# epruesse/SINA

Measured on AMD Instinct MI355X. Metric: aligned sequences/sec (whole node), 100k full-length 16S vs SILVA-NR-scale ref, higher is better.
Workload: dtype f32

## Files before the change

### sina_amd/csrc/graph_build.hip

```cpp
#include <algorithm>
#include <cstring>
#include <type_traits>

#include "common.h"
#include "ctx.h"

namespace sina_hip {
namespace {

#ifndef SINA_GRAPH_THREADS
#define SINA_GRAPH_THREADS 512
#endif
#ifndef SINA_GRAPH_MINWAVES
#define SINA_GRAPH_MINWAVES 8
#endif
constexpr int kGT = SINA_GRAPH_THREADS;
constexpr uint32_t kNoPrev = 0xFFFFu;
constexpr int kMaxFam = kFamilyMax;
constexpr int kSz = kBuiltWords;
#ifndef SINA_GRAPH_KTC
#define SINA_GRAPH_KTC 128
#endif
#ifndef SINA_GRAPH_TNW
#define SINA_GRAPH_TNW 512
#endif
constexpr int kTC = SINA_GRAPH_KTC;
constexpr int kTNW = SINA_GRAPH_TNW;
static_assert(kTC % 64 == 0 && kTC < 255 && kTNW >= 32 && kTNW % 2 == 0, "tile geometry");
static_assert((kMaxFam * (kTC / 64) + SINA_GRAPH_THREADS / 64 - 1) / (SINA_GRAPH_THREADS / 64) <= 64, "far-entry flags of a wave fit 64 bits");

#ifdef SINA_DP_PROFILE
__device__ unsigned long long g_graph_prof[16];
#define GP_DECL unsigned long long gp_[16] = {}; unsigned long long gt_ = __builtin_amdgcn_s_memtime();
#define GP(i) { const unsigned long long t_ = __builtin_amdgcn_s_memtime(); gp_[i] += t_ - gt_; gt_ = t_; }
#define GP_FLUSH if (threadIdx.x == 0) { for (int i_ = 0; i_ < 16; i_++) atomicAdd(&g_graph_prof[i_], gp_[i_]); }
#else
#define GP_DECL
#define GP(i)
#define GP_FLUSH
#endif

struct GraphArgs {
    const uint32_t *ref_ab;
    const uint64_t *ref_off;
    const uint32_t *fam_ids;
    const uint64_t *fam_off;
    const uint64_t *pred_off;
    const float *wtab;
    uint4 *rec;
    uint32_t *node_pos;
    uint32_t *succ_min;
    uint32_t *far_mark;
    uint32_t *pred;
    uint32_t *sizes;
    uint32_t width, ncap;
    uint32_t tile_bytes;
    uint32_t bitmap_off;
    uint32_t member_off;
    uint32_t member_cap;
    uint32_t fam_cap;
    int W;
    int want_smin;
    uint2 *reach;
    float kappa64;
};

struct Member {
    uint64_t beg;
    uint32_t len;
    uint32_t cur, curn;
    uint32_t carry, carryn;
    uint32_t id;
};
static_assert(sizeof(Member) == 32, "LDS layout");
constexpr uint32_t kOCpos = 0;
constexpr uint32_t kONbase = kOCpos + 4 * kTC;
constexpr uint32_t kOPres = kONbase + 4 * (kTC + 2);
constexpr uint32_t kOWA = kOPres + 4 * kTC;
constexpr uint32_t kOWC = kOWA + 4 * kTNW;
constexpr uint32_t kOWD = kOWC + 4 * kTNW;
constexpr uint32_t kOWB = (kOWD + 4 * kTNW + 7) & ~7u;
constexpr uint32_t kOLi = kOWB + 8 * kTNW;
constexpr uint32_t kONn = kOLi + 32 * kTC;
constexpr uint32_t kONfar = kONn + kTC;
constexpr uint32_t kOMask = kONfar + kTNW;
constexpr uint32_t kONcol = kOMask + kTNW;
constexpr uint32_t kOE = (kONcol + kTNW + 15) & ~15u;

template <typename In, typename Out>
__device__ uint32_t block_exscan(const In *in, Out *out, uint32_t n, uint32_t *tmp) {
    const uint32_t tid = threadIdx.x;
    const uint32_t chunk = (n + kGT - 1) / kGT;
    const uint32_t b = min(n, tid * chunk), e = min(n, b + chunk);
    uint32_t s = 0;
    for (uint32_t i = b; i < e; i++) s += (uint32_t)in[i];
    uint32_t x = s;
    const int lane = tid & 63, wave = tid >> 6;
#pragma unroll
    for (int off = 1; off < 64; off <<= 1) {
        const uint32_t y = __shfl_up(x, off);
        if (lane >= off) x += y;
    }
    if (lane == 63) tmp[wave] = x;
    __syncthreads();
    uint32_t base = 0, total = 0;
    for (int w = 0; w < kGT / 64; w++) {
        if (w < wave) base += tmp[w];
        total += tmp[w];
    }
    uint32_t run = base + x - s;
    __syncthreads();
    for (uint32_t i = b; i < e; i++) {
        const uint32_t v = (uint32_t)in[i];
        out[i] = (Out)run;
        run += v;
    }
    __syncthreads();
    return total;
}

template <typename Get, typename Out>
__device__ uint32_t block_exscan_f(uint32_t n, Get get, Out *out, uint32_t *tmp) {
    const uint32_t tid = threadIdx.x;
    const uint32_t chunk = (n + kGT - 1) / kGT;
    const uint32_t b = min(n, tid * chunk), e = min(n, b + chunk);
    uint32_t s = 0;
    for (uint32_t i = b; i < e; i++) s += get(i);
    uint32_t x = s;
    const int lane = tid & 63, wave = tid >> 6;
#pragma unroll
    for (int off = 1; off < 64; off <<= 1) {
        const uint32_t y = __shfl_up(x, off);
        if (lane >= off) x += y;
    }
    if (lane == 63) tmp[wave] = x;
    __syncthreads();
    uint32_t base = 0, total = 0;
    for (int w = 0; w < kGT / 64; w++) {
        if (w < wave) base += tmp[w];
        total += tmp[w];
    }
    uint32_t run = base + x - s;
    __syncthreads();
    for (uint32_t i = b; i < e; i++) {
        const uint32_t v = get(i);
        out[i] = (Out)run;
        run += v;
    }
    __syncthreads();
    return total;
}

__device__ __attribute__((noinline)) void fill_tile(const uint32_t *__restrict__ ref_ab, uint32_t bitmap_off, uint32_t member_off,
                                                    uint32_t nwords, uint32_t n_tasks, uint32_t c0, uint32_t tc) {
    extern __shared__ __attribute__((aligned(16))) unsigned char smem[];
    uint32_t *cposT = reinterpret_cast<uint32_t *>(smem + kOCpos);
    uint32_t *presT = reinterpret_cast<uint32_t *>(smem + kOPres);
    uint16_t *eE = reinterpret_cast<uint16_t *>(smem + kOE);
    const uint32_t *bitmap = reinterpret_cast<const uint32_t *>(smem + bitmap_off);
    const uint16_t *wrank = reinterpret_cast<const uint16_t *>(bitmap + nwords);
    Member *mb = reinterpret_cast<Member *>(smem + member_off);
    constexpr uint32_t kEAbsent = 0x00FFu, kEFirst = 1u << 13;
    constexpr uint32_t kCH = kTC / 64, kNW = kGT / 64;
    const uint32_t wave = (uint32_t)__builtin_amdgcn_readfirstlane((int)(threadIdx.x >> 6));
    const uint32_t lane = threadIdx.x & 63u;
    auto rank = [&](uint32_t pos) -> uint32_t {
        return (uint32_t)wrank[pos >> 5] + __popc(bitmap[pos >> 5] & ((1u << (pos & 31)) - 1u));
    };
        for (uint32_t t4 = wave; t4 < n_tasks; t4 += 8 * kNW) {
            uint32_t abv[8];
#pragma unroll
            for (int u = 0; u < 8; u++) {
                const uint32_t task = t4 + (uint32_t)u * kNW;
                abv[u] = 0xFFFFFFFFu;
                if (task < n_tasks) {
                    const uint32_t j = task / kCH;
                    const uint32_t cur = (uint32_t)__builtin_amdgcn_readfirstlane((int)mb[j].cur);
                    const uint32_t len = (uint32_t)__builtin_amdgcn_readfirstlane((int)mb[j].len);
                    const uint64_t beg = mb[j].beg;
                    const uint64_t begs = ((uint64_t)(uint32_t)__builtin_amdgcn_readfirstlane((int)(uint32_t)(beg >> 32)) << 32) |
                                          (uint32_t)__builtin_amdgcn_readfirstlane((int)(uint32_t)beg);
                    const uint32_t i = cur + (task % kCH) * 64u + lane;
                    if (i < len) abv[u] = ref_ab[begs + i];
                }
            }
#pragma unroll
            for (int u = 0; u < 8; u++) {
                const uint32_t task = t4 + (uint32_t)u * kNW;
                if (task >= n_tasks) continue;
                const uint32_t j = task / kCH, slot0 = (task % kCH) * 64u, slot = slot0 + lane;
                const uint32_t cur = (uint32_t)__builtin_amdgcn_readfirstlane((int)mb[j].cur);
                uint32_t ev = kEAbsent;
                if (abv[u] != 0xFFFFFFFFu) {
                    const uint32_t ab = abv[u];
                    const uint32_t pos = ab & 0xFFFFFFu;
                    const uint32_t c = rank(pos) - c0;
                    if (c < tc) {
                        const uint32_t m = (ab >> 24) & 0x1Fu;
                        ev = c | (m << 8) | (cur + slot == 0 ? kEFirst : 0u);
                        atomicOr(&presT[c], 1u << m);
                        cposT[c] = pos;
                    }
                }
                eE[j * (uint32_t)kTC + slot] = (uint16_t)ev;
                const uint32_t n_in = (uint32_t)__popcll(__builtin_amdgcn_ballot_w64(ev != kEAbsent));
                if (n_in && lane == 0) atomicMax(&mb[j].curn, cur + slot0 + n_in);
            }
        }
}

__device__ __forceinline__ uint32_t node_of_entry(uint32_t ev) {
    extern __shared__ __attribute__((aligned(16))) unsigned char smem[];
    const uint32_t *nbaseT = reinterpret_cast<const uint32_t *>(smem + kONbase);
    const uint32_t *presT = reinterpret_cast<const uint32_t *>(smem + kOPres);
    const uint8_t *liOf = smem + kOLi;
    const uint32_t c = ev & 0xFFu, m = (ev >> 8) & 31u;
    const uint32_t b = nbaseT[c];
    return b + liOf[b + __popc(presT[c] & ((1u << m) - 1u))];
}
__global__ void __launch_bounds__(kGT) __attribute__((amdgpu_waves_per_eu(SINA_GRAPH_MINWAVES, SINA_GRAPH_MINWAVES))) family_graph_kernel(GraphArgs a) {
    extern __shared__ __attribute__((aligned(16))) unsigned char smem[];
    __shared__ uint32_t s_tmp[kGT / 64 + 8];
    const uint32_t q = blockIdx.x, tid = threadIdx.x;
    const uint32_t nwords = (a.width + 31) / 32;
    const uint64_t f0 = a.fam_off[q];
    const uint32_t F = (uint32_t)(a.fam_off[q + 1] - f0);
    uint32_t *cposT = reinterpret_cast<uint32_t *>(smem + kOCpos);
    uint32_t *nbaseT = reinterpret_cast<uint32_t *>(smem + kONbase);
    uint32_t *presT = reinterpret_cast<uint32_t *>(smem + kOPres);
    uint32_t *wA = reinterpret_cast<uint32_t *>(smem + kOWA);
    uint32_t *wC = reinterpret_cast<uint32_t *>(smem + kOWC);
    uint32_t *wD = reinterpret_cast<uint32_t *>(smem + kOWD);
    unsigned long long *wB = reinterpret_cast<unsigned long long *>(smem + kOWB);
    uint8_t *liOf = smem + kOLi;
    uint8_t *nn = smem + kONn;
    uint8_t *nfarN = smem + kONfar;
    uint8_t *maskN = smem + kOMask;
    uint8_t *ncolN = smem + kONcol;
    uint16_t *eE = reinterpret_cast<uint16_t *>(smem + kOE);
    uint32_t *bitmap = reinterpret_cast<uint32_t *>(smem + a.bitmap_off);
    uint16_t *wrank = reinterpret_cast<uint16_t *>(bitmap + nwords);
    Member *mb = reinterpret_cast<Member *>(smem + a.member_off);
    constexpr uint32_t kEFirst = 1u << 13;
    constexpr uint32_t kCH = kTC / 64, kNW = kGT / 64;
    const uint32_t wave = (uint32_t)__builtin_amdgcn_readfirstlane((int)(threadIdx.x >> 6));
    const uint32_t lane = threadIdx.x & 63u;
    const uint32_t n_tasks = F * kCH;

    uint32_t *sz = a.sizes + kSz * (size_t)q;
    for (uint32_t j = tid; j < F; j += kGT) {
        const uint32_t id = a.fam_ids[f0 + j];
        mb[j].id = id;
        mb[j].beg = a.ref_off[id];
        mb[j].len = (uint32_t)(a.ref_off[id + 1] - a.ref_off[id]);
        mb[j].cur = mb[j].curn = 0;
        mb[j].carry = mb[j].carryn = kNoPrev;
    }
    for (uint32_t i = tid; i < nwords; i += kGT) bitmap[i] = 0;
    __syncthreads();
    GP_DECL

    for (uint32_t j0 = 0; j0 < F; j0 += 8) {
        uint32_t maxlen = 0;
#pragma unroll
        for (int u = 0; u < 8; u++) maxlen = max(maxlen, j0 + u < F ? mb[j0 + u].len : 0u);
        for (uint32_t i = tid; i < maxlen; i += kGT) {
            uint32_t ab[8];
#pragma unroll
            for (int u = 0; u < 8; u++)
                ab[u] = (j0 + u < F && i < mb[j0 + u].len) ? a.ref_ab[mb[j0 + u].beg + i] : 0xFFFFFFFFu;
#pragma unroll
            for (int u = 0; u < 8; u++)
                if (ab[u] != 0xFFFFFFFFu) {
                    const uint32_t pos = ab[u] & 0xFFFFFFu;
                    atomicOr(&bitmap[pos >> 5], 1u << (pos & 31));
                }
        }
    }
    __syncthreads();
    GP(0)
    {
        const uint32_t chunk = (nwords + kGT - 1) / kGT;
        const uint32_t b = min(nwords, tid * chunk), e = min(nwords, b + chunk);
        uint32_t s = 0;
        for (uint32_t i = b; i < e; i++) s += __popc(bitmap[i]);
        uint32_t x = s;
        const int lane = tid & 63, wave = tid >> 6;
#pragma unroll
        for (int off = 1; off < 64; off <<= 1) {
            const uint32_t y = __shfl_up(x, off);
            if (lane >= off) x += y;
        }
        if (lane == 63) s_tmp[wave] = x;
        __syncthreads();
        uint32_t base = 0, total = 0;
        for (int w = 0; w < kGT / 64; w++) {
            if (w < wave) base += s_tmp[w];
            total += s_tmp[w];
        }
        uint32_t run = base + x - s;
        for (uint32_t i = b; i < e; i++) {
            wrank[i] = (uint16_t)run;
            run += __popc(bitmap[i]);
        }
        if (tid == 0) s_tmp[kGT / 64] = total;
    }
    __syncthreads();
    const uint32_t NC = s_tmp[kGT / 64];
    if (NC > 65535u) {
        if (tid == 0) {
            sz[0] = NC;
            sz[1] = sz[2] = 0;
            sz[3] = 2;
        }
        return;
    }
    auto rank = [&](uint32_t pos) -> uint32_t {
        return (uint32_t)wrank[pos >> 5] + __popc(bitmap[pos >> 5] & ((1u << (pos & 31)) - 1u));
    };
    uint4 *rec = a.rec + (size_t)q * a.ncap;
    uint32_t *node_pos = a.node_pos + (size_t)q * a.ncap;
    uint32_t *smin = a.succ_min + (size_t)q * a.ncap;
    uint32_t *last = a.far_mark + (size_t)q * a.ncap;
    uint32_t *pred = a.pred + a.pred_off[q];
    const float *wt = a.wtab + (size_t)F * (kMaxFam + 1);
    uint32_t N = 0, E = 0;
    GP(1)

    for (uint32_t c0 = 0; c0 < NC; c0 += kTC) {
        const uint32_t tc = min((uint32_t)kTC, NC - c0);
        for (uint32_t i = tid; i < (uint32_t)kTC; i += kGT) presT[i] = 0;
        __syncthreads();
        GP(2)
        fill_tile(a.ref_ab, a.bitmap_off, a.member_off, nwords, n_tasks, c0, tc);
        __syncthreads();
        for (uint32_t c = tid; c < tc; c += kGT) nn[c] = (uint8_t)__popc(presT[c]);
        __syncthreads();
        GP(3)
        const uint32_t tn = block_exscan(nn, nbaseT, tc, s_tmp);
        if (tid == 0) nbaseT[tc] = tn;
        for (uint32_t ln = tid; ln < tn; ln += kGT)
            if (N + ln < a.ncap) {
                last[N + ln] = 0;
                if (a.want_smin) smin[N + ln] = 0xFFFFFFFFu;
            }
        __syncthreads();
        GP(5)
        uint32_t te = 0;
        for (uint32_t ca = 0; ca < tc;) {
            const uint32_t w0 = nbaseT[ca];
            uint32_t cb = tc;
            if (tn - w0 > (uint32_t)kTNW) {
                uint32_t lo = ca + 1, hi = tc;
                while (lo < hi) {
                    const uint32_t mid = (lo + hi + 1) / 2;
                    if (nbaseT[mid] - w0 <= (uint32_t)kTNW) lo = mid;
                    else hi = mid - 1;
                }
                cb = lo;
            }
            const uint32_t wn = nbaseT[cb] - w0;
            for (uint32_t i = tid; i < wn; i += kGT) {
                wA[i] = 0;
                wB[i] = 0;
                wC[i] = 0xFFFFFFFFu;
                nfarN[i] = 0;
            }
            __syncthreads();
            for (uint32_t task = wave; task < n_tasks; task += kNW) {
                const uint32_t j = task / kCH, slot = (task % kCH) * 64u + lane;
                const uint32_t ev = eE[j * (uint32_t)kTC + slot];
                const uint32_t c = ev & 0xFFu;
                if (c >= ca && c < cb) {
                    const uint32_t m = (ev >> 8) & 31u;
                    atomicMin(&wC[nbaseT[c] + __popc(presT[c] & ((1u << m) - 1u)) - w0], j);
                }
            }
            __syncthreads();
            for (uint32_t c = ca + tid; c < cb; c += kGT) {
                const uint32_t base = nbaseT[c], k = nn[c];
                uint32_t pp = presT[c];
                for (uint32_t x = 0; x < k; x++) {
                    const uint32_t mj = wC[base - w0 + x];
                    uint32_t r = 0;
                    for (uint32_t y = 0; y < k; y++) r += (wC[base - w0 + y] < mj) ? 1u : 0u;
                    liOf[base + x] = (uint8_t)r;
                    maskN[base - w0 + r] = (uint8_t)(__ffs(pp) - 1);
                    ncolN[base - w0 + r] = (uint8_t)c;
                    pp &= pp - 1u;
                }
            }
            __syncthreads();
            GP(4)
            auto node_of = [&](uint32_t ev) -> uint32_t { return node_of_entry(ev); };
            unsigned long long farbits = 0;
            {
                uint32_t it = 0;
                for (uint32_t task = wave; task < n_tasks; task += kNW, it++) {
                    const uint32_t j = task / kCH, slot = (task % kCH) * 64u + lane;
                    const uint32_t ev = eE[j * (uint32_t)kTC + slot];
                    const uint32_t c = ev & 0xFFu;
                    const bool mine = c >= ca && c < cb;
                    const uint32_t ln = mine ? node_of(ev) : 0u;
                    uint32_t lnp = __shfl_up(ln, 1);
                    const bool left_mine = __shfl_up(mine ? 1 : 0, 1) != 0;
                    if (!mine) continue;
                    const uint32_t node = N + ln;
                    const bool first = (ev & kEFirst) != 0;
                    atomicAdd(&wA[ln - w0], first ? 1u : 0x10001u);
                    if (mb[j].cur + slot + 1 == mb[j].curn) mb[j].carryn = node;
                    if (!first) {
                        if (slot && (lane == 0 || !left_mine)) lnp = node_of(eE[j * (uint32_t)kTC + slot - 1]);
                        const uint32_t pn = slot ? N + lnp : mb[j].carry;
                        const uint32_t d = node - pn;
                        if (d <= 64u) atomicOr(&wB[ln - w0], 1ull << (d - 1u));
                        else farbits |= 1ull << it;
                    }
                }
            }
            for (uint32_t i = tid; i < wn; i += kGT) wC[i] = 0xFFFFFFFFu;
            __syncthreads();
            GP(6)
            const uint32_t te_w = block_exscan_f(wn, [&](uint32_t i) { return wA[i] >> 16; }, wD, s_tmp);
            while (__syncthreads_or(farbits != 0 ? 1 : 0)) {
                uint32_t it = 0;
                for (uint32_t task = wave; task < n_tasks; task += kNW, it++) {
                    if (!((farbits >> it) & 1ull)) continue;
                    const uint32_t j = task / kCH, slot = (task % kCH) * 64u + lane;
                    const uint32_t ln = node_of(eE[j * (uint32_t)kTC + slot]);
                    const uint32_t pn = slot ? N + node_of(eE[j * (uint32_t)kTC + slot - 1]) : mb[j].carry;
                    atomicMin(&wC[ln - w0], pn);
                }
                __syncthreads();
                it = 0;
                for (uint32_t task = wave; task < n_tasks; task += kNW, it++) {
                    if (!((farbits >> it) & 1ull)) continue;
                    const uint32_t j = task / kCH, slot = (task % kCH) * 64u + lane;
                    const uint32_t ln = node_of(eE[j * (uint32_t)kTC + slot]);
                    const uint32_t pn = slot ? N + node_of(eE[j * (uint32_t)kTC + slot - 1]) : mb[j].carry;
                    if (wC[ln - w0] == pn) farbits &= ~(1ull << it);
                }
                __syncthreads();
                for (uint32_t i = tid; i < wn; i += kGT) {
                    const uint32_t v = wC[i];
                    if (v == 0xFFFFFFFFu) continue;
                    const uint32_t node = N + w0 + i;
                    if (node < a.ncap) {
                        pred[E + te + wD[i] + nfarN[i]] = v;
                        if (a.want_smin) atomicMin(&smin[v], cposT[ncolN[i]]);
                        atomicMax(&last[v], node);
                    }
                    nfarN[i]++;
                    wC[i] = 0xFFFFFFFFu;
                }
            }
            for (uint32_t i = tid; i < wn; i += kGT) {
                const uint32_t node = N + w0 + i;
                if (node >= a.ncap) continue;
                const uint32_t seg = E + te + wD[i];
                const uint32_t pos = cposT[ncolN[i]];
                uint32_t np = nfarN[i];
                unsigned long long bits = wB[i];
                while (bits) {
                    const uint32_t hi = 63u - (uint32_t)__clzll((long long)bits);
                    bits ^= 1ull << hi;
                    const uint32_t pa = node - (hi + 1u);
                    pred[seg + np] = pa;
                    np++;
                    if (a.want_smin) atomicMin(&smin[pa], pos);
                    atomicMax(&last[pa], node);
                }
                uint4 r;
                r.x = seg;
                r.y = __float_as_uint(wt[wA[i] & 0xFFFFu]);
                r.z = (np & 0xFFu) | ((uint32_t)maskN[i] << 8);
                r.w = kRowNone;
                rec[node] = r;
                node_pos[node] = pos;
            }
            te += te_w;
            ca = cb;
            __syncthreads();
        }
        for (uint32_t j = tid; j < F; j += kGT) {
            mb[j].cur = mb[j].curn;
            mb[j].carry = mb[j].carryn;
        }
        N += tn;
        E += te;
        __syncthreads();
        GP(7)
    }
    if (N > a.ncap || N > 65535u) {
        if (tid == 0) {
            sz[0] = N;
            sz[1] = sz[2] = 0;
            sz[3] = 2;
        }
        return;
    }
    GP(8)
    const uint32_t seg_len = dp_slot_segment(N);
    const uint32_t n_seg = (N + seg_len - 1) / seg_len;
    uint32_t *codeL = reinterpret_cast<uint32_t *>(smem);
    const bool in_lds = (size_t)N * 4 <= a.tile_bytes;
    if (tid == 0) s_tmp[kGT / 64 + 1] = 0xFFFFFFFFu;
    __syncthreads();
    for (uint32_t i = tid; i < N; i += kGT) {
        uint32_t z = rec[i].z;
        const uint32_t l = last[i];
        if (l == 0) {
            z |= kRecSink;
            atomicMin(&s_tmp[kGT / 64 + 1], i);
            if (a.want_smin) smin[i] = 1000000u;
        }
        if (l > i && l - i > (uint32_t)kFarLds) z |= kRecFence;
        rec[i].z = z;
        if (in_lds) codeL[i] = l | ((z & kRecSink) ? (1u << 30) : 0u) | ((z & kRecFence) ? (1u << 31) : 0u);
    }
    __syncthreads();
    GP(9)
    if (tid < n_seg) {
        auto walk = [&](auto kslots) {
            constexpr int K = decltype(kslots)::value;
            uint32_t fa[K];
#pragma unroll
            for (int x = 0; x < K; x++) fa[x] = (x < a.W) ? 0u : 0xFFFFFFFFu;
            uint32_t nsp = 0;
            const uint32_t b = tid * seg_len, e = min(N, b + seg_len);
            for (uint32_t m = b; m < e; m++) {
                uint32_t l, sink, fence;
                if (in_lds) {
                    const uint32_t cd = codeL[m];
                    l = cd & 0xFFFFu;
                    sink = cd & (1u << 30);
                    fence = cd & (1u << 31);
                } else {
                    const uint32_t z = rec[m].z;
                    l = last[m];
                    sink = z & kRecSink;
                    fence = z & kRecFence;
                }
                uint32_t wv = kRowNone;
                if (!sink && l != m + 1) {
                    const bool may_slot = !fence && l < e;
                    uint32_t slot = K;
#pragma unroll
                    for (int x = K - 1; x >= 0; x--) slot = (may_slot && fa[x] <= m) ? (uint32_t)x : slot;
#pragma unroll
                    for (int x = 0; x < K; x++) fa[x] = (slot == (uint32_t)x) ? l : fa[x];
                    wv = slot < (uint32_t)K ? slot : (kRowSpilled | nsp++);
                }
                if (in_lds) codeL[m] = wv;
                else rec[m].w = wv;
            }
            mb[tid].id = nsp;
        };
        if (a.W <= 4) walk(std::integral_constant<int, 4>());
        else walk(std::integral_constant<int, 8>());
    }
    __syncthreads();
    {
        uint32_t tot = 0;
        for (uint32_t g = 0; g < n_seg; g++) tot += mb[g].id;
        for (uint32_t i = tid; i < N; i += kGT) {
            uint32_t w = in_lds ? codeL[i] : rec[i].w;
            if (w != kRowNone && (w & kRowSpilled)) {
                uint32_t base = 0;
                for (uint32_t g = 0; g < i / seg_len; g++) base += mb[g].id;
                w += base;
            }
            rec[i].w = w;
            if (in_lds) codeL[i] = w;
        }
        if (tid == 0) {
            sz[0] = N;
            sz[1] = E;
            sz[2] = tot;
            sz[3] = (tot > kMaxSpillRows) ? 4u : 0u;
            sz[4] = s_tmp[kGT / 64 + 1];
        }
    }
    __syncthreads();
    GP(10)
    for (uint32_t i = tid; i < N; i += kGT) {
        const uint4 r = rec[i];
        const uint32_t np = r.z & 0xFFu;
        uint32_t first_far = 0;
        uint32_t dist = np ? 0u : kRecDistFar;
        for (uint32_t x = 0; x < np; x++) {
            const uint32_t pa = pred[r.x + x];
            uint32_t pw = in_lds ? codeL[pa] : rec[pa].w;
            if (pw == kRowNone) pw = 0;
            const bool sp = (pw & kRowSpilled) != 0;
            if (sp && first_far == 0) first_far = x + 1;
            dist = max(dist, i - pa);
            pred[r.x + x] = pa | ((pw & 0x7FFFu) << 16) | (sp ? kPredSpilled : 0u);
        }
        rec[i].z = r.z | (first_far << 24) | (min(dist, kRecDistFar) << kRecDistShift);
    }
    GP(11)
    if (a.reach != nullptr) {
        uint2 *rg = a.reach + (size_t)q * a.ncap;
        uint32_t *cw = in_lds ? codeL : (a.want_smin ? last : smin);
        if (tid == 0) s_tmp[kGT / 64 + 2] = 0xFFFFFFFFu;
        __syncthreads();
        for (uint32_t i = tid; i < N; i += kGT) {
            const uint32_t pos = node_pos[i];
            if (i > 0 && node_pos[i - 1] == pos) continue;
            uint32_t mx = 0;
            for (uint32_t j = i; j < N && node_pos[j] == pos; j++) {
                mx = max(mx, prune_gain_units(__uint_as_float(rec[j].y), a.kappa64));
                cw[j] = 0;
            }
            cw[i] = mx;
            atomicMin(&s_tmp[kGT / 64 + 2], mx);
        }
        __syncthreads();
        if (tid == 0) sz[5] = s_tmp[kGT / 64 + 2];
        const uint32_t total = block_exscan(cw, cw, N, s_tmp);
        for (uint32_t i = tid; i < N; i += kGT) {
            const uint32_t pos = node_pos[i];
            if (i > 0 && node_pos[i - 1] == pos) continue;
            const uint32_t right = (i + 1 < N) ? total - cw[i + 1] : 0u;
            const uint32_t cols_right = NC - 1u - rank(pos);
            for (uint32_t j = i; j < N && node_pos[j] == pos; j++) rg[j] = uint2{right, ((a.want_smin && !in_lds) ? 0u : last[j]) | (cols_right << 16)};
        }
    }
    GP(12)
    GP_FLUSH
}

size_t graph_bitmap_off(uint32_t max_family) { return ((size_t)kOE + 2 * (size_t)max_family * kTC + 15) & ~(size_t)15; }
size_t graph_lds_bytes(uint32_t width, uint32_t max_family) {
    const size_t nwords = (width + 31) / 32;
    return graph_bitmap_off(max_family) + ((6 * nwords + 15) & ~(size_t)15);
}
size_t graph_member_cap(uint32_t max_family) { return std::max<size_t>(16, (max_family + 1) & ~(size_t)1); }
size_t graph_lds_total(uint32_t width, uint32_t max_family) {
    return graph_lds_bytes(width, max_family) + sizeof(Member) * graph_member_cap(max_family);
}

}
}

using namespace sina_hip;

namespace {

int build_family_graphs(sina_hip_ctx *c, const uint32_t *fam_ids, const uint64_t *fam_off, uint32_t q0,
                        uint32_t bq, float fs_weight, int W, BuiltGraphs *bg, bool want_smin, float kappa64) {
    hipStream_t s = c->stream;
    if (ensure_ref_off_host(c)) return 1;
    if (!(c->wtab_fs_weight == fs_weight) || !c->g_wtab.p) {
        std::vector<float> wt((size_t)(kMaxFam + 1) * (kMaxFam + 1), 0.f);
        const float weight = fs_weight;
        for (unsigned F = 1; F <= (unsigned)kMaxFam; F++)
            for (unsigned cnt = 0; cnt <= F; cnt++)
                wt[(size_t)F * (kMaxFam + 1) + cnt] =
                    (float)(1.0 / (double)(weight + 1) + (double)(weight * ((float)cnt / (float)F)));
        if (c->g_wtab.reserve(wt.size() * 4)) return 1;
        SH_CHECK(hipMemcpyAsync(c->g_wtab.p, wt.data(), wt.size() * 4, hipMemcpyHostToDevice, s));
        SH_CHECK(hipStreamSynchronize(s));
        c->wtab_fs_weight = fs_weight;
    }
    std::vector<uint64_t> foff(bq + 1), elems(bq, 0);
    uint32_t max_f = 1;
    bg->pred_off.assign(bq, 0);
    for (uint32_t q = 0; q <= bq; q++) foff[q] = fam_off[q0 + q] - fam_off[q0];
    for (uint32_t q = 0; q < bq; q++) {
        max_f = std::max<uint32_t>(max_f, (uint32_t)(foff[q + 1] - foff[q]));
        for (uint64_t x = fam_off[q0 + q]; x < fam_off[q0 + q + 1]; x++) {
            const uint32_t id = fam_ids[x];
            if (id >= c->st->n_refs) SH_FAIL("align_families: reference id out of range");
            elems[q] += c->st->ref_off_host[id + 1] - c->st->ref_off_host[id];
        }
    }
    uint32_t ncap = std::min<uint32_t>(65535, 12288);
    for (int attempt = 0;; attempt++) {
        uint64_t pred_total = 0;
        for (uint32_t q = 0; q < bq; q++) {
            bg->pred_off[q] = pred_total;
            pred_total += elems[q] + 8;
        }
        const size_t glds_tables = graph_lds_bytes(c->st->width, max_f);
        const size_t glds = graph_lds_total(c->st->width, max_f);
        if (glds > 160 * 1024) SH_FAIL("align_families: family too wide for the device DAG build");
        if (c->g_fam_ids.reserve(4 * std::max<uint64_t>(foff[bq], 1)) || c->g_fam_off.reserve(8 * ((uint64_t)bq + 1)) ||
            c->g_tmp1.reserve(8 * (uint64_t)bq) ||
            c->rec.reserve(sizeof(uint4) * (uint64_t)bq * ncap) || c->node_pos.reserve(4 * (uint64_t)bq * ncap) ||
            c->succ_minpos.reserve(4 * (uint64_t)bq * ncap) || c->g_tmp3.reserve(4 * (uint64_t)bq * ncap) ||
            c->pred.reserve(4 * pred_total) || c->g_sizes.reserve(4 * kSz * (uint64_t)bq) ||
            (kappa64 > 0.f && c->rgain.reserve(8 * (uint64_t)bq * ncap)))
            return 1;
        if (upload(c, 1, c->g_fam_ids.p, fam_ids + fam_off[q0], 4 * foff[bq], s) ||
            upload(c, 2, c->g_fam_off.p, foff.data(), 8 * ((uint64_t)bq + 1), s) ||
            upload(c, 3, c->g_tmp1.p, bg->pred_off.data(), 8 * (uint64_t)bq, s))
            return 1;
        GraphArgs ga;
        ga.ref_ab = c->st->ref_ab.as<uint32_t>();
        ga.ref_off = c->st->ref_off.as<uint64_t>();
        ga.fam_ids = c->g_fam_ids.as<uint32_t>();
        ga.fam_off = c->g_fam_off.as<uint64_t>();
        ga.pred_off = c->g_tmp1.as<uint64_t>();
        ga.wtab = c->g_wtab.as<float>();
        ga.rec = c->rec.as<uint4>();
        ga.node_pos = c->node_pos.as<uint32_t>();
        ga.succ_min = c->succ_minpos.as<uint32_t>();
        ga.far_mark = c->g_tmp3.as<uint32_t>();
        ga.pred = c->pred.as<uint32_t>();
        ga.sizes = c->g_sizes.as<uint32_t>();
        ga.width = c->st->width;
        ga.ncap = ncap;
        ga.bitmap_off = (uint32_t)graph_bitmap_off(max_f);
        ga.tile_bytes = ga.bitmap_off;
        ga.member_off = (uint32_t)glds_tables;
        ga.member_cap = (uint32_t)graph_member_cap(max_f);
        ga.fam_cap = max_f;
        ga.W = W;
        ga.want_smin = want_smin ? 1 : 0;
        ga.reach = kappa64 > 0.f ? c->rgain.as<uint2>() : nullptr;
        ga.kappa64 = kappa64;
        if (allow_full_lds(reinterpret_cast<const void *>(family_graph_kernel))) return 1;
        bg->sizes.resize(kSz * (size_t)bq);
        {
            heavy_launch hl(c, s, kHeavyGraph);
            SH_CHECK(hipEventRecord(c->ev[6], hl.stream()));
            hipLaunchKernelGGL(family_graph_kernel, dim3(bq), dim3(kGT), glds, hl.stream(), ga);
            SH_CHECK(hipGetLastError());
            SH_CHECK(hipEventRecord(c->ev[7], hl.stream()));
            if (hl.done()) return 1;
        }
        if (download(c, 4, c->g_sizes.p, 4 * kSz * (uint64_t)bq, s)) return 1;
        SH_CHECK(wait_stream(c, s));
        memcpy(bg->sizes.data(), c->h_stage[4].p, 4 * kSz * (uint64_t)bq);
        float gms = 0;
        SH_CHECK(hipEventElapsedTime(&gms, c->ev[6], c->ev[7]));
        {
            uint64_t bytes = 0;
            for (uint32_t q = 0; q < bq; q++)
                bytes += 4 * elems[q] + (uint64_t)bg->sizes[kSz * q] * (16 + 4 + (kappa64 > 0.f ? 8 : 0)) + 4 * (uint64_t)bg->sizes[kSz * q + 1];
            std::lock_guard<std::mutex> slk(c->st->stats_mu);
            c->st->stats.graph_ms += gms;
            c->st->stats.graph_bytes += bytes;
            c->st->stats.graph_launches++;
        }
        uint32_t need_n = 0;
        for (uint32_t q = 0; q < bq; q++) {
            if (bg->sizes[kSz * q + 3] == 2) need_n = std::max(need_n, bg->sizes[kSz * q]);
            if (bg->sizes[kSz * q + 3] == 4) SH_FAIL("align_families: too many spill rows for one query");
        }
        if (!need_n) break;
        if (attempt >= 3 || need_n > 65535u) SH_FAIL("align_families: family DAG exceeds device limits");
        ncap = std::min<uint32_t>(65535, need_n + need_n / 8 + 16);
    }
    bg->ncap = ncap;
    return 0;
}

int build_graphs_for_launch(sina_hip_ctx *c, const uint32_t *fam_ids, const uint64_t *fam_off, uint32_t q0, uint32_t n,
                            const sina_hip_align_params *p, int W, const PrunePlan &pp, BuiltGraphs *bg) {
    return build_family_graphs(c, fam_ids, fam_off, q0, n, p->fs_weight, W, bg, p->insertion == SINA_INSERTION_FORBID,
                               pp.on ? pp.kappa64 : 0.f);
}

}

namespace sina_hip {

int align_family_batches(sina_hip_ctx *c, const char *who, family_builder build, bool profile_batch, const uint32_t *fam_ids,
                         const uint64_t *fam_off, uint32_t nq, const uint8_t *qmask, const uint64_t *qoff,
                         const sina_hip_align_params *p, sina_hip_align_out *out, uint32_t *out_pos) {
    const std::string w(who);
    if (!c || !fam_ids || !fam_off || !qmask || !qoff || !p || !out)
        SH_FAIL(w + ": null argument");
    std::lock_guard<std::mutex> lk(c->mu);
    sina_hip_hint_guard hints(c);
    if (!c->st->have_refs) SH_FAIL(w + ": upload references first");
    if (nq == 0) return 0;
    SH_CHECK(hipSetDevice(c->device));
    hipStream_t s = c->stream;
    if (c->st->width > 524288u) SH_FAIL(w + ": alignment wider than 524288 columns (use align_graphs)");
    if (profile_batch && p->weights != nullptr && p->n_weights > 0)
        SH_FAIL(w + ": a profile batch takes no positional weights (scoring_scheme_profile)");
    uint32_t maxL = 0;
    for (uint32_t q = 0; q < nq; q++) {
        const uint64_t L = qoff[q + 1] - qoff[q], F = fam_off[q + 1] - fam_off[q];
        if (L == 0 || L > 65535) SH_FAIL(w + ": query length must be in 1..65535");
        if (F == 0 || F > (uint64_t)kMaxFam) SH_FAIL(w + ": family size must be in 1..128");
        maxL = std::max<uint32_t>(maxL, (uint32_t)L);
    }
    DpPlan pl;
    if (plan_dp(c, maxL, &pl)) return 1;
    const int Lp = pl.geom.Lp();
    if (upload_weights(c, p)) return 1;
    if (c->h_out_pos.reserve(4 * std::max<uint64_t>(qoff[nq] - qoff[0], 1))) return 1;

    const uint64_t tb_budget_cells = tb_plane_budget(c) / tb_cell_bytes(p->insertion == SINA_INSERTION_FORBID);
    const uint32_t slots = dp_wave_slots(c, pl.geom.B);
    const uint32_t chunk_q = 3 * slots;
    BuiltGraphs bg;
    std::vector<uint32_t> dag_of;
    std::vector<uint32_t> ufam_ids;
    std::vector<uint64_t> ufam_off;
    for (uint32_t q0 = 0; q0 < nq; q0 += chunk_q) {
        const uint32_t bq = std::min(chunk_q, nq - q0);
        dag_of.assign(bq, 0);
        uint32_t n_dags = bq;
        const uint32_t *b_ids = fam_ids;
        const uint64_t *b_off = fam_off;
        uint32_t b_q0 = q0;
        if (bq > 1) {
            auto fam_hash = [&](uint32_t q) {
                uint64_t h = 0xcbf29ce484222325ull ^ (fam_off[q + 1] - fam_off[q]);
                for (uint64_t x = fam_off[q]; x < fam_off[q + 1]; x++) {
                    h = (h ^ fam_ids[x]) * 0x100000001b3ull;
                    h ^= h >> 31;
                }
                return h;
            };
            size_t cap = 16;
            while (cap < 2 * (size_t)bq) cap <<= 1;
            std::vector<uint32_t> slot(cap, 0xFFFFFFFFu), first;
            std::vector<uint64_t> hq(bq);
            for (uint32_t q = 0; q < bq; q++) {
                hq[q] = fam_hash(q0 + q);
                size_t at = (size_t)(hq[q] >> 17) & (cap - 1);
                for (;;) {
                    const uint32_t u = slot[at];
                    if (u == 0xFFFFFFFFu) {
                        slot[at] = (uint32_t)first.size();
                        dag_of[q] = (uint32_t)first.size();
                        first.push_back(q);
                        break;
                    }
                    const uint32_t f = first[u];
                    const uint64_t la = fam_off[q0 + q + 1] - fam_off[q0 + q], lb = fam_off[q0 + f + 1] - fam_off[q0 + f];
                    if (hq[f] == hq[q] && la == lb && memcmp(fam_ids + fam_off[q0 + q], fam_ids + fam_off[q0 + f], 4 * la) == 0) {
                        dag_of[q] = u;
                        break;
                    }
                    at = (at + 1) & (cap - 1);
                }
            }
            n_dags = (uint32_t)first.size();
            if (n_dags < bq) {
                ufam_off.assign((size_t)n_dags + 1, 0);
                for (uint32_t u = 0; u < n_dags; u++)
                    ufam_off[u + 1] = ufam_off[u] + (fam_off[q0 + first[u] + 1] - fam_off[q0 + first[u]]);
                ufam_ids.resize(ufam_off[n_dags]);
                for (uint32_t u = 0; u < n_dags; u++)
                    memcpy(ufam_ids.data() + ufam_off[u], fam_ids + fam_off[q0 + first[u]], 4 * (ufam_off[u + 1] - ufam_off[u]));
                b_ids = ufam_ids.data();
                b_off = ufam_off.data();
                b_q0 = 0;
            } else {
                for (uint32_t q = 0; q < bq; q++) dag_of[q] = q;
            }
        } else {
            for (uint32_t q = 0; q < bq; q++) dag_of[q] = q;
        }
        PrunePlan pp;
        if (!profile_batch)
            pp = prune_plan(p, (float)(1.0 / (double)(p->fs_weight + 1) + (double)p->fs_weight), p->fs_weight >= 0.f ? 0.f : -1.f, maxL, false);
        if (build(c, b_ids, b_off, b_q0, n_dags, p, pl.W, pp, &bg)) return 1;
        {
            std::lock_guard<std::mutex> slk(c->st->stats_mu);
            c->st->stats.dags_built += n_dags;
            c->st->stats.dags_used += bq;
        }
        uint32_t r0 = 0;
        while (r0 < bq) {
            uint32_t r1 = r0;
            uint64_t tbc = 0, sprows = 0, cells = 0;
            uint32_t erec_cursor = 0;
            std::vector<QDesc> qd;
            std::vector<uint32_t> chain_ref;
            while (r1 < bq) {
                const uint32_t u = dag_of[r1];
                const uint32_t N = bg.sizes[kSz * u];
                if (r1 > r0 && tbc + (uint64_t)N * Lp > tb_budget_cells) break;
                QDesc d;
                d.node_off = (uint64_t)u * bg.ncap;
                d.edge_off = bg.pred_off[u];
                d.q_off = qoff[q0 + r1] - qoff[q0 + r0];
                d.tb_off = tbc;
                d.spill_off = sprows;
                d.N = N;
                d.L = (uint32_t)(qoff[q0 + r1 + 1] - qoff[q0 + r1]);
                d.n_spill = bg.sizes[kSz * u + 2];
                d.first_sink = bg.sizes[kSz * u + 4];
                d.gmin = bg.sizes[kSz * u + 5];
                d.erec_off = erec_cursor;
                erec_cursor += dp_edge_entries(N);
                qd.push_back(d);
                chain_ref.push_back(fam_ids[fam_off[q0 + r1]]);
                tbc += (uint64_t)N * Lp;
                sprows += d.n_spill;
                cells += (uint64_t)N * d.L;
                r1++;
            }
            {
                const uint32_t r1r = dp_round_range(r0, r1, bq, slots);
                for (uint32_t r = r1r; r < r1; r++) {
                    tbc -= (uint64_t)qd[r - r0].N * Lp;
                    sprows -= qd[r - r0].n_spill;
                    cells -= (uint64_t)qd[r - r0].N * qd[r - r0].L;
                }
                qd.resize(r1r - r0);
                chain_ref.resize(r1r - r0);
                r1 = r1r;
            }
            const uint32_t rq = r1 - r0;
            const uint64_t qbase = qoff[q0 + r0], nqm = qoff[q0 + r1] - qbase;
            if (c->qd.reserve(sizeof(QDesc) * rq) || c->qmask.reserve(std::max<uint64_t>(nqm, 1))) return 1;
            if (upload(c, 5, c->qd.p, qd.data(), sizeof(QDesc) * rq, s) || upload(c, 6, c->qmask.p, qmask + qbase, nqm, s))
                return 1;
            c->profile_batch = profile_batch;
            c->out_pos_base = qbase - qoff[0];
            if (run_dp_device(c, pl, qd.data(), rq, (uint64_t)n_dags * bg.ncap, tbc, sprows, cells, nqm, p, c->st->width,
                              out + q0 + r0, out_pos ? out_pos + qbase : nullptr, false, pp, profile_batch ? nullptr : chain_ref.data()))
                return 1;
            r0 = r1;
        }
    }
    return 0;
}

}

extern "C" {

int sina_hip_align_families(sina_hip_ctx *c, const uint32_t *fam_ids, const uint64_t *fam_off, uint32_t nq,
                            const uint8_t *qmask, const uint64_t *qoff, const sina_hip_align_params *p,
                            sina_hip_align_out *out, uint32_t *out_pos) {
    return align_family_batches(c, "align_families", build_graphs_for_launch, false, fam_ids, fam_off, nq, qmask, qoff, p, out, out_pos);
}

#ifdef SINA_DP_PROFILE
int sina_hip_debug_graph_profile(unsigned long long *out16, int reset) {
    SH_CHECK(hipMemcpyFromSymbol(out16, HIP_SYMBOL(g_graph_prof), sizeof(unsigned long long) * 16));
    if (reset) {
        unsigned long long z[16] = {};
        SH_CHECK(hipMemcpyToSymbol(HIP_SYMBOL(g_graph_prof), z, sizeof z));
    }
    return 0;
}
#endif

int sina_hip_debug_family_graph(sina_hip_ctx *c, const uint32_t *fam_ids, uint32_t F, float fs_weight,
                                uint32_t ring_depth, uint32_t *n_nodes, uint32_t *n_edges, uint32_t *pos,
                                uint8_t *mask, float *weight, uint32_t *pred_off, uint32_t *pred,
                                uint32_t *succ_minpos, uint8_t *sink, uint32_t *spill_idx, uint32_t cap_nodes,
                                uint32_t cap_edges) {
    if (!c || !fam_ids || !n_nodes || !n_edges) SH_FAIL("debug_family_graph: null argument");
    std::lock_guard<std::mutex> lk(c->mu);
    if (!c->st->have_refs) SH_FAIL("debug_family_graph: upload references first");
    if (F == 0 || F > (uint32_t)kMaxFam) SH_FAIL("debug_family_graph: family size must be in 1..128");
    SH_CHECK(hipSetDevice(c->device));
    const uint64_t foff[2] = {0, F};
    BuiltGraphs bg;
    if (build_family_graphs(c, fam_ids, foff, 0, 1, fs_weight, (int)ring_depth, &bg, true, fs_weight >= 0.f ? 64.0f * 1.0001f * 2.0f : 0.f)) return 1;
    const uint32_t N = bg.sizes[0];
    std::vector<uint4> rec(N);
    std::vector<uint32_t> pr(bg.sizes[1] + 8);
    SH_CHECK(hipMemcpy(rec.data(), c->rec.p, sizeof(uint4) * N, hipMemcpyDeviceToHost));
    SH_CHECK(hipMemcpy(pr.data(), c->pred.p, 4 * pr.size(), hipMemcpyDeviceToHost));
    uint32_t E = 0;
    for (uint32_t m = 0; m < N; m++) E += rec[m].z & 0xffu;
    *n_nodes = N;
    *n_edges = E;
    if (N > cap_nodes || E > cap_edges) SH_FAIL("debug_family_graph: output buffers too small");
    SH_CHECK(hipMemcpy(pos, c->node_pos.p, 4 * N, hipMemcpyDeviceToHost));
    SH_CHECK(hipMemcpy(succ_minpos, c->succ_minpos.p, 4 * N, hipMemcpyDeviceToHost));
    uint32_t e = 0;
    for (uint32_t m = 0; m < N; m++) {
        mask[m] = (uint8_t)((rec[m].z >> 8) & 0xffu);
        memcpy(&weight[m], &rec[m].y, 4);
        sink[m] = (rec[m].z & kRecSink) ? 1 : 0;
        spill_idx[m] = rec[m].w;
        pred_off[m] = e;
        for (uint32_t x = 0; x < (rec[m].z & 0xffu); x++) pred[e++] = pr[rec[m].x + x] & 0xffffu;
    }
    pred_off[N] = e;
    return 0;
}

}
```

Measured before the change: 276,400.

## Overlap reach-bound maxima with slot walk and precompute slot predicates

Precomputes kept/may-slot flags into the LDS code word so the serial per-segment slot walk does fewer branches, and software-pipelines that walk with 8-wide LDS prefetch. When the reach array fits beside the code array in LDS, the per-column prune-gain maxima are computed by non-walking waves while wave 0 runs the serial walk, removing two barriers. Also prefetches predecessor indices, writes z and w together, and simplifies the reach fill to per-node. This adds LDS usage and more intricate indexing, and running the atomicMin in the overlapped path could race if wave assumptions don't hold.

```diff
diff --git a/sina_amd/csrc/graph_build.hip b/sina_amd/csrc/graph_build.hip
--- a/sina_amd/csrc/graph_build.hip
+++ b/sina_amd/csrc/graph_build.hip
@@ -504,7 +504,12 @@
     const uint32_t n_seg = (N + seg_len - 1) / seg_len;
     uint32_t *codeL = reinterpret_cast<uint32_t *>(smem);
     const bool in_lds = (size_t)N * 4 <= a.tile_bytes;
-    if (tid == 0) s_tmp[kGT / 64 + 1] = 0xFFFFFFFFu;
+    const bool beside = a.reach != nullptr && (size_t)N * 8 <= a.tile_bytes;
+    constexpr uint32_t kCodeKept = 1u << 30, kCodeMaySlot = 1u << 31;
+    if (tid == 0) {
+        s_tmp[kGT / 64 + 1] = 0xFFFFFFFFu;
+        s_tmp[kGT / 64 + 2] = 0xFFFFFFFFu;
+    }
     __syncthreads();
     for (uint32_t i = tid; i < N; i += kGT) {
         uint32_t z = rec[i].z;
@@ -516,43 +521,74 @@
         }
         if (l > i && l - i > (uint32_t)kFarLds) z |= kRecFence;
         rec[i].z = z;
-        if (in_lds) codeL[i] = l | ((z & kRecSink) ? (1u << 30) : 0u) | ((z & kRecFence) ? (1u << 31) : 0u);
+        if (in_lds) {
+            const bool kept = l != 0 && l != i + 1;
+            const uint32_t seg_end = min(N, (i / seg_len + 1u) * seg_len);
+            codeL[i] = l | (kept ? kCodeKept : 0u) | ((kept && !(z & kRecFence) && l < seg_end) ? kCodeMaySlot : 0u);
+        }
     }
     __syncthreads();
     GP(9)
+    auto bound_maxima = [&](uint32_t *cw, uint32_t t0, uint32_t nt) {
+        for (uint32_t i = t0; i < N; i += nt) {
+            const uint32_t pos = node_pos[i];
+            uint32_t mx = 0;
+            if (i == 0 || node_pos[i - 1] != pos) {
+                uint32_t j = i;
+                do mx = max(mx, prune_gain_units(__uint_as_float(rec[j].y), a.kappa64));
+                while (++j < N && node_pos[j] == pos);
+                atomicMin(&s_tmp[kGT / 64 + 2], mx);
+            }
+            cw[i] = mx;
+        }
+    };
+    if (beside && wave != 0) bound_maxima(codeL + N, tid - 64u, (uint32_t)kGT - 64u);
     if (tid < n_seg) {
         auto walk = [&](auto kslots) {
             constexpr int K = decltype(kslots)::value;
-            uint32_t fa[K];
-#pragma unroll
-            for (int x = 0; x < K; x++) fa[x] = (x < a.W) ? 0u : 0xFFFFFFFFu;
+            int32_t fa[K];
+#pragma unroll
+            for (int x = 0; x < K; x++) fa[x] = (x < a.W) ? 0 : 0x7FFFFFFF;
             uint32_t nsp = 0;
             const uint32_t b = tid * seg_len, e = min(N, b + seg_len);
-            for (uint32_t m = b; m < e; m++) {
-                uint32_t l, sink, fence;
-                if (in_lds) {
-                    const uint32_t cd = codeL[m];
-                    l = cd & 0xFFFFu;
-                    sink = cd & (1u << 30);
-                    fence = cd & (1u << 31);
-                } else {
-                    const uint32_t z = rec[m].z;
-                    l = last[m];
-                    sink = z & kRecSink;
-                    fence = z & kRecFence;
-                }
-                uint32_t wv = kRowNone;
-                if (!sink && l != m + 1) {
-                    const bool may_slot = !fence && l < e;
-                    uint32_t slot = K;
-#pragma unroll
-                    for (int x = K - 1; x >= 0; x--) slot = (may_slot && fa[x] <= m) ? (uint32_t)x : slot;
-#pragma unroll
-                    for (int x = 0; x < K; x++) fa[x] = (slot == (uint32_t)x) ? l : fa[x];
-                    wv = slot < (uint32_t)K ? slot : (kRowSpilled | nsp++);
-                }
-                if (in_lds) codeL[m] = wv;
-                else rec[m].w = wv;
+            auto place = [&](uint32_t m, uint32_t l, bool kept, bool may_slot) -> uint32_t {
+                const int32_t mm = may_slot ? (int32_t)m : -1;
+                uint32_t slot = K;
+#pragma unroll
+                for (int x = K - 1; x >= 0; x--) slot = (fa[x] <= mm) ? (uint32_t)x : slot;
+#pragma unroll
+                for (int x = 0; x < K; x++) fa[x] = (slot == (uint32_t)x) ? (int32_t)l : fa[x];
+                const bool spill = kept && slot == (uint32_t)K;
+                const uint32_t wv = !kept ? kRowNone : (spill ? (kRowSpilled | nsp) : slot);
+                nsp += spill ? 1u : 0u;
+                return wv;
+            };
+            if (in_lds) {
+                constexpr uint32_t G = 8;
+                auto code = [&](uint32_t m, uint32_t cd) -> uint32_t {
+                    return place(m, cd & 0xFFFFu, (cd & kCodeKept) != 0, (cd & kCodeMaySlot) != 0);
+                };
+                uint32_t cd[G], nx[G], wv[G];
+#pragma unroll
+                for (uint32_t u = 0; u < G; u++) cd[u] = codeL[min(b + u, e - 1u)];
+                uint32_t m0 = b;
+                for (; m0 + G <= e; m0 += G) {
+#pragma unroll
+                    for (uint32_t u = 0; u < G; u++) nx[u] = codeL[min(m0 + G + u, e - 1u)];
+#pragma unroll
+                    for (uint32_t u = 0; u < G; u++) wv[u] = code(m0 + u, cd[u]);
+#pragma unroll
+                    for (uint32_t u = 0; u < G; u++) codeL[m0 + u] = wv[u];
+#pragma unroll
+                    for (uint32_t u = 0; u < G; u++) cd[u] = nx[u];
+                }
+                for (; m0 < e; m0++) codeL[m0] = code(m0, codeL[m0]);
+            } else {
+                for (uint32_t m = b; m < e; m++) {
+                    const uint32_t z = rec[m].z, l = last[m];
+                    const bool kept = !(z & kRecSink) && l != m + 1;
+                    rec[m].w = place(m, l, kept, kept && !(z & kRecFence) && l < e);
+                }
             }
             mb[tid].id = nsp;
         };
@@ -570,8 +606,8 @@
                 for (uint32_t g = 0; g < i / seg_len; g++) base += mb[g].id;
                 w += base;
             }
-            rec[i].w = w;
             if (in_lds) codeL[i] = w;
+            else rec[i].w = w;
         }
         if (tid == 0) {
             sz[0] = N;
@@ -588,43 +624,41 @@
         const uint32_t np = r.z & 0xFFu;
         uint32_t first_far = 0;
         uint32_t dist = np ? 0u : kRecDistFar;
-        for (uint32_t x = 0; x < np; x++) {
-            const uint32_t pa = pred[r.x + x];
+        auto entry = [&](uint32_t x, uint32_t pa) {
             uint32_t pw = in_lds ? codeL[pa] : rec[pa].w;
             if (pw == kRowNone) pw = 0;
             const bool sp = (pw & kRowSpilled) != 0;
             if (sp && first_far == 0) first_far = x + 1;
             dist = max(dist, i - pa);
             pred[r.x + x] = pa | ((pw & 0x7FFFu) << 16) | (sp ? kPredSpilled : 0u);
-        }
-        rec[i].z = r.z | (first_far << 24) | (min(dist, kRecDistFar) << kRecDistShift);
+        };
+        constexpr uint32_t kAhead = 4;
+        uint32_t pa4[kAhead];
+#pragma unroll
+        for (uint32_t x = 0; x < kAhead; x++) pa4[x] = x < np ? pred[r.x + x] : 0u;
+#pragma unroll
+        for (uint32_t x = 0; x < kAhead; x++)
+            if (x < np) entry(x, pa4[x]);
+        for (uint32_t x = kAhead; x < np; x++) entry(x, pred[r.x + x]);
+        const uint32_t z = r.z | (first_far << 24) | (min(dist, kRecDistFar) << kRecDistShift);
+        if (in_lds) *reinterpret_cast<uint2 *>(&rec[i].z) = uint2{z, codeL[i]};
+        else rec[i].z = z;
     }
     GP(11)
     if (a.reach != nullptr) {
         uint2 *rg = a.reach + (size_t)q * a.ncap;
-        uint32_t *cw = in_lds ? codeL : (a.want_smin ? last : smin);
-        if (tid == 0) s_tmp[kGT / 64 + 2] = 0xFFFFFFFFu;
-        __syncthreads();
-        for (uint32_t i = tid; i < N; i += kGT) {
-            const uint32_t pos = node_pos[i];
-            if (i > 0 && node_pos[i - 1] == pos) continue;
-            uint32_t mx = 0;
-            for (uint32_t j = i; j < N && node_pos[j] == pos; j++) {
-                mx = max(mx, prune_gain_units(__uint_as_float(rec[j].y), a.kappa64));
-                cw[j] = 0;
-            }
-            cw[i] = mx;
-            atomicMin(&s_tmp[kGT / 64 + 2], mx);
-        }
-        __syncthreads();
+        uint32_t *cw = beside ? codeL + N : (in_lds ? codeL : (a.want_smin ? last : smin));
+        if (!beside) {
+            __syncthreads();
+            bound_maxima(cw, tid, (uint32_t)kGT);
+            __syncthreads();
+        }
         if (tid == 0) sz[5] = s_tmp[kGT / 64 + 2];
         const uint32_t total = block_exscan(cw, cw, N, s_tmp);
         for (uint32_t i = tid; i < N; i += kGT) {
-            const uint32_t pos = node_pos[i];
-            if (i > 0 && node_pos[i - 1] == pos) continue;
             const uint32_t right = (i + 1 < N) ? total - cw[i + 1] : 0u;
-            const uint32_t cols_right = NC - 1u - rank(pos);
-            for (uint32_t j = i; j < N && node_pos[j] == pos; j++) rg[j] = uint2{right, ((a.want_smin && !in_lds) ? 0u : last[j]) | (cols_right << 16)};
+            const uint32_t cols_right = NC - 1u - rank(node_pos[i]);
+            rg[i] = uint2{right, ((a.want_smin && !in_lds) ? 0u : last[i]) | (cols_right << 16)};
         }
     }
     GP(12)
```

Result: slower. 272,000 (-1.6%).

## Compute per-column prune gains during build and overlap bound writes with slot walk

Applied to the files above, without the earlier changes.

Per-column maximum prune gains are now computed inside the column-tile loop and stashed in the reach buffer, so the tail scans NC columns instead of N nodes. The prefix scan and bound writes run on waves 1+ while wave 0 does the slot-assignment walk, using a shuffle prefix sum in place of a serial spill-base loop. Sink and fence bits are folded into the final rec.z write, which drops a pass. First-writer atomicMin is skipped for columns with a single member. This adds LDS pressure (N+NC words) and relies on the reach buffer temporarily holding column gains before they are overwritten.

```diff
diff --git a/sina_amd/csrc/graph_build.hip b/sina_amd/csrc/graph_build.hip
--- a/sina_amd/csrc/graph_build.hip
+++ b/sina_amd/csrc/graph_build.hip
@@ -207,6 +207,21 @@
                 if (n_in && lane == 0) atomicMax(&mb[j].curn, cur + slot0 + n_in);
             }
         }
+}
+
+__device__ __forceinline__ void column_gains(uint32_t *__restrict__ colw, const float *__restrict__ wt, float kappa64,
+                                                       uint32_t ca, uint32_t cb, uint32_t w0, uint32_t node_cap) {
+    extern __shared__ __attribute__((aligned(16))) unsigned char smem[];
+    const uint32_t *nbaseT = reinterpret_cast<const uint32_t *>(smem + kONbase);
+    const uint32_t *wA = reinterpret_cast<const uint32_t *>(smem + kOWA);
+    const uint8_t *nn = smem + kONn;
+    for (uint32_t c = ca + threadIdx.x; c < cb; c += kGT) {
+        const uint32_t base = nbaseT[c];
+        if (base >= node_cap) continue;
+        uint32_t mx = 0;
+        for (uint32_t x = 0; x < nn[c]; x++) mx = max(mx, prune_gain_units(wt[wA[base - w0 + x] & 0xFFFFu], kappa64));
+        colw[c] = mx;
+    }
 }
 
 __device__ __forceinline__ uint32_t node_of_entry(uint32_t ev) {
@@ -372,8 +387,11 @@
                 const uint32_t ev = eE[j * (uint32_t)kTC + slot];
                 const uint32_t c = ev & 0xFFu;
                 if (c >= ca && c < cb) {
-                    const uint32_t m = (ev >> 8) & 31u;
-                    atomicMin(&wC[nbaseT[c] + __popc(presT[c] & ((1u << m) - 1u)) - w0], j);
+                    const uint32_t pp = presT[c];
+                    if (pp & (pp - 1u)) {
+                        const uint32_t m = (ev >> 8) & 31u;
+                        atomicMin(&wC[nbaseT[c] + __popc(pp & ((1u << m) - 1u)) - w0], j);
+                    }
                 }
             }
             __syncthreads();
@@ -478,6 +496,8 @@
                 rec[node] = r;
                 node_pos[node] = pos;
             }
+            if (a.reach != nullptr)
+                column_gains(reinterpret_cast<uint32_t *>(a.reach + (size_t)q * a.ncap) + c0, wt, a.kappa64, ca, cb, w0, N < a.ncap ? a.ncap - N : 0u);
             te += te_w;
             ca = cb;
             __syncthreads();
@@ -501,33 +521,60 @@
     }
     GP(8)
     const uint32_t seg_len = dp_slot_segment(N);
-    const uint32_t n_seg = (N + seg_len - 1) / seg_len;
     uint32_t *codeL = reinterpret_cast<uint32_t *>(smem);
     const bool in_lds = (size_t)N * 4 <= a.tile_bytes;
-    if (tid == 0) s_tmp[kGT / 64 + 1] = 0xFFFFFFFFu;
-    __syncthreads();
+    uint2 *rg = a.reach ? a.reach + (size_t)q * a.ncap : nullptr;
+    const bool col_lds = rg != nullptr && ((size_t)N + NC) * 4 <= a.tile_bytes;
+    uint32_t *colL = codeL + N;
+    if (tid == 0) {
+        s_tmp[kGT / 64 + 1] = 0xFFFFFFFFu;
+        s_tmp[kGT / 64 + 2] = 0xFFFFFFFFu;
+    }
+    __syncthreads();
+    auto fetch_cols = [&](uint32_t *cs) {
+        const uint32_t *colw = reinterpret_cast<const uint32_t *>(rg);
+        uint32_t mn = 0xFFFFFFFFu;
+        for (uint32_t c = tid; c < NC; c += kGT) {
+            const uint32_t v = colw[c];
+            cs[c] = v;
+            mn = min(mn, v);
+        }
+        if (mn != 0xFFFFFFFFu) atomicMin(&s_tmp[kGT / 64 + 2], mn);
+    };
+    auto write_bound = [&](const uint32_t *cs, uint32_t total, uint32_t t0, uint32_t nt) {
+        for (uint32_t j = t0; j < N; j += nt) {
+            const uint32_t col = rank(node_pos[j]);
+            const uint32_t right = (col + 1 < NC) ? total - cs[col + 1] : 0u;
+            rg[j] = uint2{right, ((a.want_smin && !in_lds) ? 0u : last[j]) | ((NC - 1u - col) << 16)};
+        }
+    };
     for (uint32_t i = tid; i < N; i += kGT) {
-        uint32_t z = rec[i].z;
         const uint32_t l = last[i];
-        if (l == 0) {
-            z |= kRecSink;
+        const bool sink = l == 0;
+        if (sink) {
             atomicMin(&s_tmp[kGT / 64 + 1], i);
             if (a.want_smin) smin[i] = 1000000u;
         }
-        if (l > i && l - i > (uint32_t)kFarLds) z |= kRecFence;
-        rec[i].z = z;
-        if (in_lds) codeL[i] = l | ((z & kRecSink) ? (1u << 30) : 0u) | ((z & kRecFence) ? (1u << 31) : 0u);
-    }
+        const bool fence = l > i && l - i > (uint32_t)kFarLds;
+        if (in_lds) codeL[i] = l | (sink ? (1u << 30) : 0u) | (fence ? (1u << 31) : 0u);
+    }
+    if (col_lds) fetch_cols(colL);
     __syncthreads();
     GP(9)
-    if (tid < n_seg) {
-        auto walk = [&](auto kslots) {
+    uint32_t col_total = 0;
+    if (col_lds) {
+        col_total = block_exscan(colL, colL, NC, s_tmp);
+        if (tid == 0) sz[5] = s_tmp[kGT / 64 + 2];
+    }
+    GP(12)
+    if (wave == 0) {
+        auto walk = [&](auto kslots) -> uint32_t {
             constexpr int K = decltype(kslots)::value;
             uint32_t fa[K];
 #pragma unroll
             for (int x = 0; x < K; x++) fa[x] = (x < a.W) ? 0u : 0xFFFFFFFFu;
             uint32_t nsp = 0;
-            const uint32_t b = tid * seg_len, e = min(N, b + seg_len);
+            const uint32_t b = min(N, tid * seg_len), e = min(N, b + seg_len);
             for (uint32_t m = b; m < e; m++) {
                 uint32_t l, sink, fence;
                 if (in_lds) {
@@ -536,10 +583,9 @@
                     sink = cd & (1u << 30);
                     fence = cd & (1u << 31);
                 } else {
-                    const uint32_t z = rec[m].z;
                     l = last[m];
-                    sink = z & kRecSink;
-                    fence = z & kRecFence;
+                    sink = l == 0 ? 1u : 0u;
+                    fence = (l > m && l - m > (uint32_t)kFarLds) ? 1u : 0u;
                 }
                 uint32_t wv = kRowNone;
                 if (!sink && l != m + 1) {
@@ -554,37 +600,40 @@
                 if (in_lds) codeL[m] = wv;
                 else rec[m].w = wv;
             }
-            mb[tid].id = nsp;
+            return nsp;
         };
-        if (a.W <= 4) walk(std::integral_constant<int, 4>());
-        else walk(std::integral_constant<int, 8>());
-    }
-    __syncthreads();
-    {
-        uint32_t tot = 0;
-        for (uint32_t g = 0; g < n_seg; g++) tot += mb[g].id;
+        const uint32_t nsp = (a.W <= 4) ? walk(std::integral_constant<int, 4>()) : walk(std::integral_constant<int, 8>());
+        uint32_t x = nsp;
+#pragma unroll
+        for (int off = 1; off < 16; off <<= 1) {
+            const uint32_t y = __shfl_up(x, off);
+            if (lane >= (uint32_t)off) x += y;
+        }
+        if (tid < 16) mb[tid].id = x - nsp;
+        if (tid == 15) s_tmp[kGT / 64 + 3] = x;
+    } else if (col_lds) {
+        write_bound(colL, col_total, tid - 64u, (uint32_t)kGT - 64u);
+    }
+    __syncthreads();
+    if (tid == 0) {
+        const uint32_t tot = s_tmp[kGT / 64 + 3];
+        sz[0] = N;
+        sz[1] = E;
+        sz[2] = tot;
+        sz[3] = (tot > kMaxSpillRows) ? 4u : 0u;
+        sz[4] = s_tmp[kGT / 64 + 1];
+    }
+    if (!in_lds) {
         for (uint32_t i = tid; i < N; i += kGT) {
-            uint32_t w = in_lds ? codeL[i] : rec[i].w;
-            if (w != kRowNone && (w & kRowSpilled)) {
-                uint32_t base = 0;
-                for (uint32_t g = 0; g < i / seg_len; g++) base += mb[g].id;
-                w += base;
-            }
-            rec[i].w = w;
-            if (in_lds) codeL[i] = w;
-        }
-        if (tid == 0) {
-            sz[0] = N;
-            sz[1] = E;
-            sz[2] = tot;
-            sz[3] = (tot > kMaxSpillRows) ? 4u : 0u;
-            sz[4] = s_tmp[kGT / 64 + 1];
-        }
-    }
-    __syncthreads();
+            const uint32_t w = rec[i].w;
+            if (w != kRowNone && (w & kRowSpilled)) rec[i].w = w + mb[i / seg_len].id;
+        }
+        __syncthreads();
+    }
     GP(10)
     for (uint32_t i = tid; i < N; i += kGT) {
         const uint4 r = rec[i];
+        const uint32_t l = last[i];
         const uint32_t np = r.z & 0xFFu;
         uint32_t first_far = 0;
         uint32_t dist = np ? 0u : kRecDistFar;
@@ -593,41 +642,32 @@
             uint32_t pw = in_lds ? codeL[pa] : rec[pa].w;
             if (pw == kRowNone) pw = 0;
             const bool sp = (pw & kRowSpilled) != 0;
+            if (sp && in_lds) pw += mb[pa / seg_len].id;
             if (sp && first_far == 0) first_far = x + 1;
             dist = max(dist, i - pa);
             pred[r.x + x] = pa | ((pw & 0x7FFFu) << 16) | (sp ? kPredSpilled : 0u);
         }
-        rec[i].z = r.z | (first_far << 24) | (min(dist, kRecDistFar) << kRecDistShift);
+        const uint32_t z = r.z | (l == 0 ? kRecSink : 0u) | ((l > i && l - i > (uint32_t)kFarLds) ? kRecFence : 0u) |
+                           (first_far << 24) | (min(dist, kRecDistFar) << kRecDistShift);
+        if (in_lds) {
+            uint32_t w = codeL[i];
+            if (w != kRowNone && (w & kRowSpilled)) w += mb[i / seg_len].id;
+            *reinterpret_cast<uint2 *>(&rec[i].z) = uint2{z, w};
+        } else {
+            rec[i].z = z;
+        }
     }
     GP(11)
-    if (a.reach != nullptr) {
-        uint2 *rg = a.reach + (size_t)q * a.ncap;
+    if (rg != nullptr && !col_lds) {
         uint32_t *cw = in_lds ? codeL : (a.want_smin ? last : smin);
-        if (tid == 0) s_tmp[kGT / 64 + 2] = 0xFFFFFFFFu;
         __syncthreads();
-        for (uint32_t i = tid; i < N; i += kGT) {
-            const uint32_t pos = node_pos[i];
-            if (i > 0 && node_pos[i - 1] == pos) continue;
-            uint32_t mx = 0;
-            for (uint32_t j = i; j < N && node_pos[j] == pos; j++) {
-                mx = max(mx, prune_gain_units(__uint_as_float(rec[j].y), a.kappa64));
-                cw[j] = 0;
-            }
-            cw[i] = mx;
-            atomicMin(&s_tmp[kGT / 64 + 2], mx);
-        }
+        fetch_cols(cw);
         __syncthreads();
+        const uint32_t total = block_exscan(cw, cw, NC, s_tmp);
         if (tid == 0) sz[5] = s_tmp[kGT / 64 + 2];
-        const uint32_t total = block_exscan(cw, cw, N, s_tmp);
-        for (uint32_t i = tid; i < N; i += kGT) {
-            const uint32_t pos = node_pos[i];
-            if (i > 0 && node_pos[i - 1] == pos) continue;
-            const uint32_t right = (i + 1 < N) ? total - cw[i + 1] : 0u;
-            const uint32_t cols_right = NC - 1u - rank(pos);
-            for (uint32_t j = i; j < N && node_pos[j] == pos; j++) rg[j] = uint2{right, ((a.want_smin && !in_lds) ? 0u : last[j]) | (cols_right << 16)};
-        }
-    }
-    GP(12)
+        write_bound(cw, total, tid, (uint32_t)kGT);
+    }
+    GP(13)
     GP_FLUSH
 }
 
```

Measured after the change: 273,900 before, 270,400 after. 1.3% lower.
